# PriviligedLearningDistributedAerial/imitation

Hardware: AMD Instinct MI355X
Metric: env-steps/sec (whole node) + final eval return, GAIL HalfCheetah-v4 at 1/2/4/8 MI355X (higher is better)
Workload: dtype mixed (fp32 master weights and accumulation; PPO products as split-bf16 x3 ~fp32, discriminator bf16); 1 GPU; model=GAIL: FeedForward32Policy[32,32]+RunningNorm / BasicRewardNet(32,32)+RunningNorm, global_batch=4096, seq_len=512, parallelism=dp1, engine=device, env=HalfCheetah-v4

## Files before the change

csrc/bind/engine.cpp:

```cpp
#include "common.h"
#include "launchers.h"
#include "vec_env.h"

namespace {

template <typename T>
T* tptr(const py::dict& d, const char* k, bool optional = false) {
  if (!d.contains(k) || d[k].is_none()) {
    TORCH_CHECK(optional, "engine arg missing: ", k);
    return nullptr;
  }
  auto t = d[k].cast<torch::Tensor>();
  TORCH_CHECK(t.is_cuda() && t.is_contiguous(), "engine arg ", k, " must be a contiguous GPU tensor");
  return reinterpret_cast<T*>(t.data_ptr());
}

int ival(const py::dict& d, const char* k, int def = 0) { return d.contains(k) ? d[k].cast<int>() : def; }
double fval(const py::dict& d, const char* k, double def = 0.0) { return d.contains(k) ? d[k].cast<double>() : def; }

ia::WaveMLP wave_mlp(const py::dict& d) {
  ia::WaveMLP m{};
  auto Ws = d["W"].cast<std::vector<torch::Tensor>>();
  auto bs = d["b"].cast<std::vector<torch::Tensor>>();
  TORCH_CHECK(!Ws.empty() && Ws.size() <= (size_t)ia::kWaveMaxLayers, "1..4 layers");
// ... 280 lines not shown
  return o;
}

std::string ppo_row(py::dict d) {
  ia::PPORcPlan plan;
  return ppo_plan_rc(d, plan) ? std::string(plan.row->name) : "lds";
}

size_t ppo_lds(py::dict d) { return ia::ppo_lds_bytes(ppo_shape_args(d)); }

torch::Tensor ppo_image_probe(torch::Tensor x, int mode) {
  TORCH_CHECK(x.is_cuda() && x.scalar_type() == torch::kFloat32 && x.dim() == 2 && x.is_contiguous(),
              "engine_ppo_image_probe: a contiguous fp32 [rows][features] device matrix");
  const int rows = (int)x.size(0), feats = (int)x.size(1);
  TORCH_CHECK(rows > 0 && rows <= 64 && rows % 16 == 0 && feats > 0 && feats <= 64 && feats % 16 == 0,
              "engine_ppo_image_probe: rows and features multiples of 16, at most 64");
  TORCH_CHECK(mode == 0 || mode == 1, "engine_ppo_image_probe: mode 0 (packed store) or 1 (per element)");
  auto out = torch::zeros({2, feats / 16, (rows > 32 ? 64 : 32) / 32, 64, 8}, x.options().dtype(torch::kInt16));
  IA_HIP_CHECK(ia::ppo_image_probe_launch(x.data_ptr<float>(), rows, feats, mode,
                                           reinterpret_cast<unsigned short*>(out.data_ptr<int16_t>()), ia_stream()));
  return out;
}

}

void dagger_env_step(py::dict d) {
  ia::DaggerEnvArgs a{};
  std::string env = d["env"].cast<std::string>();
  int ms = 0;
  TORCH_CHECK(ia::make_env_params(env, &a.P, &ms), "unknown native env ", env);
  a.N = ival(d, "N");
  a.max_steps = ival(d, "max_steps", ms);
  a.mode = ival(d, "mode", 0);
  a.sdim = ia::state_size(a.P);
  a.state = tptr<float>(d, "state");
  a.rng = tptr<uint64_t>(d, "rng");
  a.elapsed = tptr<int>(d, "elapsed");
  a.ep_ret = tptr<float>(d, "ep_ret");
  auto check_numel = [&](const char* k, int64_t want) {
    if (!d.contains(k) || d[k].is_none()) return;
    auto t = d[k].cast<torch::Tensor>();
    TORCH_CHECK(t.numel() == want, "dagger_env_step: ", k, " has ", t.numel(), " elements, expected ", want);
  };
  check_numel("state", (int64_t)a.N * a.sdim);
  check_numel("rng", a.N);
  check_numel("elapsed", a.N);
// ... 25 lines not shown
    for (const char* k : {"rew", "term", "trunc", "ep_ret_out", "ep_len_out"}) check_numel(k, a.N);
    if (d.contains("obs_rec") && !d["obs_rec"].is_none()) {
      a.obs_rec = img ? (void*)tptr<uint8_t>(d, "obs_rec") : (void*)tptr<float>(d, "obs_rec");
      check_numel("obs_rec", a.N * obs_elems);
    }
  }
  IA_HIP_CHECK(ia::dagger_env_step(a, ia_stream()));
}

void register_engine(py::module& m) {
  m.def("dagger_env_step", &dagger_env_step, "DAgger collector: one device env step (mode 0) / reset all (mode 1)");
  m.def("engine_rollout", &rollout, "T-step device rollout (actor sampling + env) for N envs");
  m.def("engine_rollout_post", &rollout_post,
        "values, log-probs, TimeLimit bootstrap and learned reward of a rollout, all transitions in parallel");
  m.def("engine_reward_outnorm", &reward_outnorm, "NormalizedRewardNet output normalisation over a rollout");
  m.def("engine_reward_retnorm", &reward_retnorm, "VecNormalize discounted-return reward normalisation over a rollout");
  m.def("engine_ppo_update", &ppo_update, "persistent PPO update / DP minibatch grads / apply");
  m.def("engine_ppo_path", &ppo_path, "kernel used by engine_ppo_update mode 0 (rc | lds)");
  m.def("engine_ppo_row", &ppo_row, "instance-table row that engine_ppo_update mode 0 runs (lean or full; lds off the fast path)");
  m.def("engine_ppo_plan", &ppo_plan, "host plan of the register-chained PPO update: instance + launch geometry");
  m.def("engine_ppo_lds", &ppo_lds, "LDS bytes the PPO kernel needs for a configuration");
  m.def("engine_ppo_image_probe", &ppo_image_probe,
        "dW operand fragments of a matrix through the PPO update's split-bf16 image store and transposed reads (test hook)");
}
```

csrc/include/ia/wave.h:

```cpp
#pragma once
#include <hip/hip_runtime.h>
#include <stdint.h>

#include "ia/common.h"
#include "ia/mfma.h"
#include "ia/rng.h"

namespace ia {

typedef __attribute__((address_space(3))) float lf;
typedef float f32v4 __attribute__((ext_vector_type(4)));
typedef __attribute__((address_space(3))) f32v4 lf4;
typedef __attribute__((address_space(3))) int li;

__device__ __forceinline__ void wave_sync() {
  __builtin_amdgcn_fence(__ATOMIC_RELEASE, "wavefront");
  __builtin_amdgcn_wave_barrier();
  __builtin_amdgcn_fence(__ATOMIC_ACQUIRE, "wavefront");
}

__device__ __forceinline__ float bcast(float v, int k) {
  return __int_as_float(__builtin_amdgcn_readlane(__float_as_int(v), k));
}


template <int CTRL>
__device__ __forceinline__ float dpp(float v) {
  return __int_as_float(__builtin_amdgcn_update_dpp(0, __float_as_int(v), CTRL, 0xF, 0xF, true));
}
__device__ __forceinline__ float sum_lanes8(float v) {
  v += dpp<0xB1>(v);
  v += dpp<0x4E>(v);
  v += dpp<0x114>(v);
  return bcast(v, 7);
}

__device__ __forceinline__ float row_sum16(float v) {
  v += dpp<0xB1>(v);
  v += dpp<0x4E>(v);
  v += dpp<0x141>(v);
  v += dpp<0x140>(v);
  return v;
}
__device__ __forceinline__ float row_max16(float v) {
  v = fmaxf(v, dpp<0xB1>(v));
  v = fmaxf(v, dpp<0x4E>(v));
  v = fmaxf(v, dpp<0x141>(v));
  v = fmaxf(v, dpp<0x140>(v));
  return v;
}

__device__ __forceinline__ float add_rows16(float v) {
  const auto r = __builtin_amdgcn_permlane16_swap(__float_as_uint(v), __float_as_uint(v), false, false);
  return __uint_as_float(r[0]) + __uint_as_float(r[1]);
}
__device__ __forceinline__ float max_rows16(float v) {
  const auto r = __builtin_amdgcn_permlane16_swap(__float_as_uint(v), __float_as_uint(v), false, false);
  return fmaxf(__uint_as_float(r[0]), __uint_as_float(r[1]));
}
__device__ __forceinline__ float max_halves(float v) {
  const auto r = __builtin_amdgcn_permlane32_swap(__float_as_uint(v), __float_as_uint(v), false, false);
  return fmaxf(__uint_as_float(r[0]), __uint_as_float(r[1]));
}

__device__ __forceinline__ float add_halves(float v) {
  const auto r = __builtin_amdgcn_permlane32_swap(__float_as_uint(v), __float_as_uint(v), false, false);
// ... 28 lines not shown
```

csrc/kernels/launchers.h:

```cpp
#pragma once
#include <hip/hip_runtime.h>
#include <stddef.h>
#include <stdint.h>

#include "ia/engine.h"
#include "ia/tmlp.h"

namespace ia {

int tmlp_waves_for(const MLPDesc& d, int static_lds = 0);
size_t tmlp_slab_floats(const MLPDesc& d, int B);
hipError_t tmlp_forward(const MLPDesc& d, const float* X, int B, float* Y, hipStream_t s);
hipError_t tmlp_backward(const MLPDesc& d, const float* X, const float* dY, int B, float* dX, const MLPGrads& g,
                         float* slab, hipStream_t s);

int tmlp_disc_blocks(const MLPDesc& d, int B);
hipError_t tmlp_disc_fwd_bwd(const MLPDesc& d, const float* X, int B, const DiscLoss& dl, float* slab, hipStream_t s);

struct TransitionSrc {
  const float *obs, *next_obs, *acts;
  const int64_t* acts_i;
  const bool* dones;
};
struct RewardInputLayout {
// ... 382 lines not shown

bool rollout_split_form(const WaveMLP& m);
size_t rollout_lds_bytes(const RolloutArgs& a);
hipError_t rollout_launch(const RolloutArgs& a, hipStream_t s);
size_t rollout_post_lds_bytes(const RolloutPostArgs& a);
hipError_t rollout_post_launch(const RolloutPostArgs& a, hipStream_t s);
hipError_t reward_outnorm_launch(const OutNormArgs& a, hipStream_t s);
struct RetNormArgs {
  int T, N;
  const float* env_rew;
  const float* dones;
  const float* boot;
  float* rewards;
  double* ret;
  double* rms;
  double* work;
  double gamma, eps, clip;
};
hipError_t reward_retnorm_launch(const RetNormArgs& a, hipStream_t s);

bool ppo_rc_plan(const PPOArgs& a, PPORcPlan& plan);
hipError_t ppo_rc_launch(const PPOArgs& a, const PPORcPlan& plan, float* workspace, hipStream_t s);
hipError_t ppo_image_probe_launch(const float* x, int rows, int feats, int mode, unsigned short* out, hipStream_t s);

size_t ppo_lds_bytes(const PPOArgs& a);
hipError_t ppo_launch(const PPOArgs& a, hipStream_t s);

struct ConvGeo {
  int B, H, W, C;
  int KH, KW, S;
  int OH, OW, N;
  int P;
  int Kp;
};
bool conv_geo_ok(const ConvGeo& g);
constexpr int kMaxPack = 8;
struct ConvPackLayer {
  const float* w;
  void* wb;
  void* wt;
  int N, C, KH, KW;
  int t_hwc;
};
struct ConvPackArgs {
  ConvPackLayer layer[kMaxPack];
  int n;
// ... 80 lines not shown
```

csrc/kernels/ppo_rc.hip:

```cpp
#include <stdio.h>

#include "ppo_rc_kernel.h"
#include "ppo_rc_instances.h"

namespace ia {
namespace rc {

IA_RC_TABLE(IA_RC_EXTERN)

constexpr int kPrepWaves = 16;
constexpr int kPrepBatch = 16;

__device__ __forceinline__ int prep_idx(const PPOArgs& a, const PPORcGeo& g, int e, int mb, int c, int lane) {
  const int Bg = g.G * g.nch * g.cw;
  return a.perm[(size_t)e * a.rows + (size_t)mb * Bg + (size_t)c * g.cw + lane];
}

__global__ __launch_bounds__(64 * kPrepWaves) void ppo_rc_prep_kernel(PPOArgs a, PPORcGeo g) {
  __shared__ float red[kPrepWaves][64];
  __shared__ float stat[2][64];
  __shared__ float adv_stat[2];
  __shared__ float red_a[kPrepWaves];
  const int k = blockIdx.x;
  const int lane = threadIdx.x & 63, wv = threadIdx.x >> 6, nw = blockDim.x >> 6;
// ... 129 lines not shown
        bf16x4 hi, lo;
        split4(v, hi, lo);
        img_store4(L, 0, rp, t, st, hi, lo);
      }
    } else {
      for (int s = 0; s < feats / 4; ++s) img_store1(L, 0, rp, 4 * s + kk, row, x[(size_t)row * feats + 4 * s + kk]);
    }
  }
  __syncthreads();
  int t0, t1;
  img_lane_terms(r16, kk, t0, t1);
  const int n = T * ksteps;
  for (int i = gw; i < n; i += 4) {
    const int t = i / ksteps, ks = i - t * ksteps;
    const lch* p = (const lch*)L + t * img_strip(rp) + kImgKStep * ks + t0;
    const bf16x8 hi = img_read8(p, p + (t1 - t0));
    const bf16x8 lo = img_read8(p + img_lo(rp), p + img_lo(rp) + (t1 - t0));
    bf16x8* oh = reinterpret_cast<bf16x8*>(out) + (size_t)i * 64 + lane;
    oh[0] = hi;
    oh[(size_t)n * 64] = lo;
  }
}

}

using namespace rc;

hipError_t ppo_image_probe_launch(const float* x, int rows, int feats, int mode, unsigned short* out, hipStream_t s) {
  if (rows <= 0 || rows > kProbeMaxRows || rows % 16 != 0 || feats <= 0 || feats > kProbeMaxFeats || feats % 16 != 0 ||
      (mode != 0 && mode != 1))
    return hipErrorInvalidValue;
  hipLaunchKernelGGL(ppo_image_probe_kernel, dim3(1), dim3(256), 0, s, x, rows, feats, mode, out);
  return hipGetLastError();
}

static const PPORcRow kRcRows[] = {IA_RC_TABLE(IA_RC_ROW)};

static bool rc_row_bf3(const PPORcRow& r) { return rc_is_bf3(r.KT, r.S0T, r.NLT, r.HWT, r.CWT, r.NW); }

static const PPORcRow* rc_select(const PPOArgs& a, int kt, int cw, bool ns, bool bf3_ok, bool lean_ok) {
  const int s0 = (a.D + 3) / 4;
  for (const PPORcRow& r : kRcRows) {
    bool ok = r.ns == (int)ns && r.KT == kt && (r.CWT <= 0 || r.CWT == cw) && (lean_ok || !r.LEAN);
    ok = ok && (r.NLT <= 0 || (a.n_pi == r.NLT && a.n_vf == r.NLT));
    if (r.HWT > 0) {
      for (int l = 1; l < a.n_pi; ++l) ok = ok && a.pi_dims[l] == r.HWT;
      for (int l = 1; l < a.n_vf; ++l) ok = ok && a.vf_dims[l] == r.HWT;
    }
    ok = ok && (r.S0T > 0 ? s0 == r.S0T : (r.S0T == 0 || s0 <= -r.S0T));
// ... 228 lines not shown
```

csrc/kernels/ppo_rc_kernel.h:

```cpp
#pragma once
#include <hip/hip_runtime.h>
#include <stdlib.h>

#include "ia/engine.h"
#include "ia/wave.h"
#include "launchers.h"


namespace ia {
namespace rc {


typedef float f4 __attribute__((ext_vector_type(4)));
typedef __bf16 bf16;
typedef __bf16 bf16x8 __attribute__((ext_vector_type(8)));
typedef __attribute__((address_space(3))) bf16 lbf;
typedef __attribute__((address_space(3))) bf16x8 lbf8;
typedef __attribute__((address_space(3))) float lf;
typedef __attribute__((address_space(3))) f4 lf4;

constexpr int kL = kWaveMaxLayers;

__device__ __forceinline__ f4 mfma(float a, float b, f4 c) { return __builtin_amdgcn_mfma_f32_16x16x4f32(a, b, c, 0, 0, 0); }
__device__ __forceinline__ int rfl(int v) { return __builtin_amdgcn_readfirstlane(v); }
// ... 2 lines not shown
  const float e = __expf(2.f * fminf(fmaxf(x, -15.f), 15.f));
  return 1.f - 2.f * __builtin_amdgcn_rcpf(e + 1.f);
}

__device__ __forceinline__ float act_fn(int act, float x) {
  switch (act) {
    case 1: return fmaxf(x, 0.f);
    case 2: return tanh_fast(x);
    case 3: return x > 0.f ? x : 0.01f * x;
    case 4: return 1.f / (1.f + expf(-x));
    default: return x;
  }
}
__device__ __forceinline__ float act_grad(int act, float y) {
  switch (act) {
    case 1: return y > 0.f ? 1.f : 0.f;
    case 2: return 1.f - y * y;
    case 3: return y > 0.f ? 1.f : 0.01f;
    case 4: return y * (1.f - y);
    default: return 1.f;
  }
}
__device__ __forceinline__ float sum16(float v) { return row_sum16(v); }
__device__ __forceinline__ float sum_kk(float v) { return add_halves(add_rows16(v)); }
__device__ __forceinline__ float max_kk(float v) { return max_halves(max_rows16(v)); }

__device__ __forceinline__ void st_sc1_x4(float* p, f4 v) {
  asm volatile("global_store_dwordx4 %0, %1, off sc1" ::"v"(p), "v"(v) : "memory");
}
__device__ __forceinline__ void st_sc1_x1(float* p, float v) {
  asm volatile("global_store_dword %0, %1, off sc1" ::"v"(p), "v"(v) : "memory");
}
__device__ __forceinline__ f4 ld_sc1_x4(const float* p) {
  f4 v;
  asm volatile("global_load_dwordx4 %0, %1, off sc1" : "=v"(v) : "v"(p) : "memory");
  return v;
}
__device__ __forceinline__ void wait_vm4(f4& a, f4& b, f4& c, f4& d) {
  asm volatile("s_waitcnt vmcnt(0)" : "+v"(a), "+v"(b), "+v"(c), "+v"(d)::"memory");
}
__device__ __forceinline__ void wait_vm8(f4 (&v)[8]) {
  asm volatile("s_waitcnt vmcnt(0)"
               : "+v"(v[0]), "+v"(v[1]), "+v"(v[2]), "+v"(v[3]), "+v"(v[4]), "+v"(v[5]), "+v"(v[6]), "+v"(v[7])::"memory");
}
template <int N>
__device__ __forceinline__ void wait_vm_n(f4 (&v)[N]) {
// ... 25 lines not shown
__device__ __forceinline__ void spin_give_up(const PPOArgs& a, unsigned* tflag) {
  atomicOr(tflag, 1u);
  if (a.err) atomicOr(a.err, 1u);
}

struct LG {
  int din, dout, w, ldw, b, h, ldh, z, ldz, db;
};
__device__ __forceinline__ LG lg(const PPORcGeo& g, int q, int l) {
  LG r;
  r.din = rfl(g.din[q][l]);
  r.dout = rfl(g.dout[q][l]);
  r.w = rfl(g.w_off[q][l]);
  r.ldw = rfl(g.ldw[q][l]);
  r.b = rfl(g.b_off[q][l]);
  r.h = rfl(g.h_off[q][l]);
  r.ldh = rfl(g.ldh[q][l]);
  r.z = rfl(g.z_off[q][l]);
  r.ldz = rfl(g.ldz[q][l]);
  r.db = rfl(g.db_off[q][l]);
  return r;
}

template <int S0M>
struct Rows {
  float x[S0M];
  f4 act;
  f4 rd;
};

template <int S0M>
__device__ __forceinline__ void load_rows(const PPORcGeo& g, size_t slot, int row, int kk, int s0, Rows<S0M>& r) {
  const float* xr = g.xraw + (slot * 64 + row) * g.dp;
#pragma unroll
  for (int s = 0; s < S0M; ++s)
    if (s < s0) r.x[s] = xr[4 * s + kk];
  const float* ac = g.acts + (slot * 64 + row) * 16;
  r.act = *reinterpret_cast<const f4*>(ac + 4 * kk);
  r.rd = *reinterpret_cast<const f4*>(g.rowd + (slot * 64 + row) * 4);
}

template <int GT, int KI, int NF = 16>
__device__ __forceinline__ void exchange_sum(const float* slab, int n_items, const int (&ids)[KI], int lane, f4 (&xg)[KI]) {
  constexpr int IB0 = NF / GT;
  constexpr int IB = IB0 < KI ? IB0 : KI;
#pragma unroll
// ... 42 lines not shown
    if (rid[r] < 0) continue;
    f4 sacc = v[r * GT];
#pragma unroll
    for (int gi = 1; gi < GT; ++gi) sacc += v[r * GT + gi];
    st_sc1_x4(red + (size_t)rid[r] * 256 + lane * 4, sacc);
  }
}

typedef __bf16 bf16x4 __attribute__((ext_vector_type(4)));
typedef __attribute__((address_space(3))) bf16x4 lbf4;
typedef __attribute__((address_space(3))) char lch;

__host__ __device__ __forceinline__ int img_lo(int rp) { return 32 * rp; }
__host__ __device__ __forceinline__ int img_strip(int rp) { return 64 * rp; }
__host__ __device__ __forceinline__ int img_unit(int row, int p) {
  return 32 * (row ^ ((row >> 1) & 4)) + 8 * (p ^ ((row >> 2) & 3));
}
__device__ __forceinline__ void img_lane_terms(int r16, int kk, int& t0, int& t1) {
  t0 = img_unit(8 * kk + (r16 >> 2), r16 & 3);
  t1 = img_unit(8 * kk + 4 + (r16 >> 2), r16 & 3);
}
constexpr int kImgKStep = 32 * 32;

__device__ __forceinline__ void split4(const f4 v, bf16x4& hi, bf16x4& lo) {
#pragma clang fp contract(off)
#pragma unroll
  for (int j = 0; j < 4; ++j) {
    const bf16 h = (bf16)v[j];
    hi[j] = h;
    lo[j] = (bf16)(v[j] - (float)h);
  }
}
__device__ __forceinline__ bf16x8 cat4(bf16x4 a, bf16x4 b) { return __builtin_shufflevector(a, b, 0, 1, 2, 3, 4, 5, 6, 7); }

__device__ __forceinline__ void img_store4(lf* L, int off, int rp, int t, int st, bf16x4 hi, bf16x4 lo) {
  lch* p = (lch*)L + 4 * off + t * img_strip(rp) + st;
  *(lbf4*)p = hi;
  *(lbf4*)(p + img_lo(rp)) = lo;
}
__device__ __forceinline__ void img_store1(lf* L, int off, int rp, int f, int row, float v) {
  lch* p = (lch*)L + 4 * off + (f >> 4) * img_strip(rp) + img_unit(row, (f >> 2) & 3) + 2 * (f & 3);
  const bf16 h = (bf16)v;
  *(lbf*)p = h;
  *(lbf*)(p + img_lo(rp)) = (bf16)(v - (float)h);
}
__device__ __forceinline__ bf16x8 img_read8(const lch* a0, const lch* a1) {
  const bf16x4 x = __builtin_amdgcn_ds_read_tr16_b64_v4bf16((lbf4*)a0);
  const bf16x4 y = __builtin_amdgcn_ds_read_tr16_b64_v4bf16((lbf4*)a1);
  return cat4(x, y);
}

__device__ __forceinline__ f4 mfma_bf16(bf16x8 a, bf16x8 b, f4 c) { return __builtin_amdgcn_mfma_f32_16x16x32_bf16(a, b, c, 0, 0, 0); }

template <int N>
// ... 10 lines not shown
        const lch* zp = Lb + izo[i0 + i] + kImgKStep * ks;
        const lch* hp = Lb + iho[i0 + i] + kImgKStep * ks;
        zh[i] = img_read8(zp, zp + d1);
        zl[i] = img_read8(zp + lo, zp + lo + d1);
        hh[i] = img_read8(hp, hp + d1);
        hl[i] = img_read8(hp + lo, hp + lo + d1);
      }
#pragma unroll
      for (int i = 0; i < GS; ++i) {
        if (i0 + i >= N) continue;
        acc[i0 + i] = mfma_bf16(zh[i], hh[i], acc[i0 + i]);
        acc[i0 + i] = mfma_bf16(zh[i], hl[i], acc[i0 + i]);
        acc[i0 + i] = mfma_bf16(zl[i], hh[i], acc[i0 + i]);
      }
    }
  }
}

__host__ __device__ __forceinline__ int bf3_ld(int k) { return k + 8; }
__device__ __forceinline__ int bf3_pos_in0(int f) { return 8 * (f & 3) + (f >> 2); }
__device__ __forceinline__ int bf3_pos_h(int f) { return 32 * (f >> 5) + 8 * ((f >> 2) & 3) + 4 * ((f >> 4) & 1) + (f & 3); }

__device__ __forceinline__ void split8(const float (&v)[8], bf16x8& hi, bf16x8& lo) {
#pragma unroll
  for (int j = 0; j < 8; ++j) {
    const bf16 h = (bf16)v[j];
    hi[j] = h;
    lo[j] = (bf16)(v[j] - (float)h);
  }
}

__device__ __forceinline__ f4 bf3_tile(const lbf* a, int lo_off, bf16x8 bh, bf16x8 bl, f4 acc) {
  const bf16x8 ah = *(const lbf8*)a;
  const bf16x8 al = *(const lbf8*)(a + lo_off);
  acc = mfma_bf16(ah, bh, acc);
  acc = mfma_bf16(ah, bl, acc);
  return mfma_bf16(al, bh, acc);
}

__device__ __forceinline__ f4 bf3_mm(bf16x8 ah, bf16x8 al, bf16x8 bh, bf16x8 bl, f4 acc) {
  acc = mfma_bf16(ah, bh, acc);
  acc = mfma_bf16(ah, bl, acc);
  return mfma_bf16(al, bh, acc);
}

template <int KT>
__device__ __forceinline__ void bf3_store_w(lf* L, const PPORcGeo& g, int q, int l, int o, int i, float v, int nl) {
  const bf16 h = (bf16)v;
  const bf16 lo = (bf16)(v - (float)h);
  const int kin = l == 0 ? 32 : 16 * KT;
  const int rows = (g.dout[q][l] + 15) & ~15;
  lbf* wf = (lbf*)(L + g.wf_off[q][l]) + o * bf3_ld(kin) + (l == 0 ? bf3_pos_in0(i) : bf3_pos_h(i));
  wf[0] = h;
  wf[rows * bf3_ld(kin)] = lo;
  if (l > 0) {
    const int kout = l == nl - 1 ? 32 : 16 * KT;
    const int trows = (g.din[q][l] + 15) & ~15;
    lbf* wt = (lbf*)(L + g.wt_off[q][l]) + i * bf3_ld(kout) + bf3_pos_h(o);
    wt[0] = h;
    wt[trows * bf3_ld(kout)] = lo;
  }
}

template <int KT>
__device__ __forceinline__ void bf3_store_tile(lf* L, int kind, int wf, int wfl, int wt, int wtl, int r16, int kk,
                                               const float (&v)[4]) {
  typedef __bf16 bf16x4 __attribute__((ext_vector_type(4)));
  typedef __attribute__((address_space(3))) bf16x4 lbf4;
  bf16x4 h4, l4;
#pragma unroll
  for (int j = 0; j < 4; ++j) {
    const bf16 h = (bf16)v[j];
    h4[j] = h;
    l4[j] = (bf16)(v[j] - (float)h);
  }
  lbf* Lb = (lbf*)L;
  const int ldi = kind == 0 ? bf3_ld(32) : bf3_ld(16 * KT);
  lbf* pf = Lb + wf + 4 * kk * ldi + (kind == 0 ? 8 * (r16 & 3) + (r16 >> 2) : 8 * (r16 >> 2) + (r16 & 3));
#pragma unroll
  for (int j = 0; j < 4; ++j) {
    pf[j * ldi] = h4[j];
    pf[j * ldi + wfl] = l4[j];
  }
  if (kind != 0) {
    const int ldo = kind == 2 ? bf3_ld(32) : bf3_ld(16 * KT);
    lbf* pt = Lb + wt + r16 * ldo + 8 * kk;
    *(lbf4*)pt = h4;
    *(lbf4*)(pt + wtl) = l4;
  }
}

constexpr bool rc_is_bf3(int KT, int S0T, int NLT, int HWT, int CWT, int NW) {
  return HWT == 16 * KT && NLT == 3 && S0T != 0 && (S0T > 0 ? S0T : -S0T) <= 8 && CWT == 64 && (NW == 4 || KT == 2);
}

template <int KT, int KW, int KB, int S0T, int NLT, int ACTT, int HWT, int CWT, int DT, int NW, int LEAN = 0>
__global__ __launch_bounds__(64 * NW) void ppo_rc_kernel(PPOArgs a, PPORcGeo g) {
  constexpr int KI = KW + KB;
// ... 8 lines not shown
  const int w = rfl(tid >> 6), lane = tid & 63;
  const int r16 = lane & 15, kk = lane >> 4;
  const bool ns = g.ns != 0;
  int bid = (int)blockIdx.x;
  if (g.xcd > 1) {
    if (bid % g.xcd) return;
    bid /= g.xcd;
  }
  const int q = ns ? (bid & 1) : w / kHalf;
  const int gw = ns ? w : w % kHalf;
  const int grp = ns ? (bid >> 1) : bid;
  const int G = kLean ? 1 : g.G, nch = g.nch, cw = CWT > 0 ? CWT : g.cw;
  const int CH = G * nch;
  const int Bg = CH * cw;
  const int RT = cw / 16;
  const bool rows_wave = gw < RT;
  const int nl = NLT > 0 ? NLT : (q == 0 ? a.n_pi : a.n_vf);
  const int D = a.D, A = a.A;
  constexpr int S0M = S0T > 0 ? S0T : (S0T < 0 ? -S0T : 16);
  const int s0 = S0T > 0 ? S0T : (D + 3) / 4;
  constexpr bool BF3 = rc_is_bf3(KT, S0T, NLT, HWT, CWT, NW);
  constexpr bool kOffPath = KB == 1 && NW == 4;
  constexpr bool kNormBatch = kOffPath && S0T > 0 && KW <= 8;
  const bool gauss = DT >= 0 ? DT == 0 : !a.discrete;
  const bool has_ls = gauss && a.log_std_off >= 0;
  float am[4];
#pragma unroll
  for (int j = 0; j < 4; ++j) am[j] = 4 * (lane >> 4) + j < a.A ? 1.f : 0.f;
  const int n_mb = a.rows / Bg;
  const int K = a.n_epochs * n_mb;
  const float invB = 1.f / (float)Bg;
  const float c_half_log2pi = 0.91893853320467274f;
  const int n_items = rfl(g.n_items);

  for (int i = tid; i < g.lds_floats; i += kThreads) L[i] = 0.f;
  __syncthreads();
#pragma unroll
  for (int qq = 0; qq < 2; ++qq) {
#pragma unroll
    for (int l = 0; l < kL; ++l) {
      if (l >= (qq == 0 ? a.n_pi : a.n_vf) || (ns && qq != q)) continue;
      const LG y = lg(g, qq, l);
      const int wo = qq == 0 ? a.pi_w_off[l] : a.vf_w_off[l];
      const int bo = qq == 0 ? a.pi_b_off[l] : a.vf_b_off[l];
      for (int i = tid; i < y.dout * y.din; i += kThreads) {
        const int o = i / y.din, c = i - o * y.din;
// ... 157 lines not shown
    if (w + ib * kWaves >= nbq) continue;
    const int desc = rfl(g.items[bb + w + ib * kWaves]);
    const int iq = desc & 1, il = (desc >> 1) & 3, kind = (desc >> 3) & 3;
    const LG y = lg(g, iq, il);
    bkind[ib] = kind;
    b_off[ib] = kind == 1 ? y.db : g.lsp_off;
    const bool ok = kind == 1 ? (lane < y.dout) : (has_ls && lane < A);
    b_okf[ib] = ok ? 1.f : 0.f;
    if (ok) b_addr[ib] = kind == 1 ? y.b + lane : g.ls_off + lane;
  }
  float pre_m = 0.f, pre_v = 0.f;
  constexpr int kAhead = kOffPath ? 2 : 1;
  if (norm_lane && K > kAhead) {
    pre_m = g.mom[kAhead * 128 + nc];
    pre_v = g.mom[kAhead * 128 + 64 + nc];
  }
  Rows<S0M> cur;
  const int row = 16 * gw + r16;
  const int sterm = img_unit(row, kk);
  auto slot_of = [&](int u) -> size_t { return (size_t)(u / nch) * CH + (size_t)grp * nch + (u % nch); };
  if (rows_wave && K > 0) load_rows(g, slot_of(0), row, kk, s0, cur);
  __shared__ unsigned long long sprof[20];
  if (tid < 20) sprof[tid] = 0;
  unsigned* arrive = g.sync + (ns ? 4 * q : 0);
  unsigned* tflag = g.sync + 1;
  unsigned* arrive2 = g.sync + (ns ? 4 * q + 2 : 2);
  const unsigned spin_lim = a.spin_limit ? a.spin_limit : (1u << 22);
  const bool stall = a.debug_stall != 0 && bid == (ns ? 2 * G : G) - 1;
  __syncthreads();

  auto norm_rows = [&](int nbuf, float (&xo)[S0M]) {
    float nmv[S0M], nrv[S0M];
#pragma unroll
    for (int s = 0; s < S0M; ++s) {
      if constexpr (kNormBatch) {
        nmv[s] = L[g.nm_off + nbuf + 4 * s + kk];
        nrv[s] = L[g.nm_off + nbuf + 64 + 4 * s + kk];
      } else {
        nmv[s] = 0.f;
        nrv[s] = 1.f;
        if (s < s0 && a.has_norm) {
          nmv[s] = L[g.nm_off + nbuf + 4 * s + kk];
          nrv[s] = L[g.nm_off + nbuf + 64 + 4 * s + kk];
        }
      }
    }
#pragma unroll
    for (int s = 0; s < S0M; ++s) xo[s] = s < s0 ? (cur.x[s] - nmv[s]) * nrv[s] : 0.f;
    if (q == 0 || ns) {
      const int h0 = rfl(g.h_off[0][0]);
#pragma unroll
      for (int s = 0; s < S0M; ++s)
        if (s < s0) img_store1(L, h0, rp, 4 * s + kk, row, xo[s]);
    }
  };
  constexpr bool PREC = KW <= 8;
  const bool pre = PREC && (ns || G > 1) && (kLean || g.xstash < 0);
  float xpre[PREC ? S0M : 1];
#pragma unroll
  for (int s = 0; s < (PREC ? S0M : 1); ++s) xpre[s] = 0.f;
  auto pre_rows = [&](int k) {
    if constexpr (PREC)
      if (pre && rows_wave && k + 1 < K) norm_rows(((k + 1) & 1) * 128, xpre);
  };

  constexpr bool kEarly = KW <= 8;
  float step_size = 0.f, inv_bc2s = 0.f;
  auto adam_scalars = [&]() {
    step += 1.f;
    b1t *= a.beta1;
    b2t *= a.beta2;
    step_size = a.lr / (1.f - b1t);
    inv_bc2s = 1.f / sqrtf(1.f - b2t);
  };

  constexpr bool PREF = BF3 && KT == 2 && NW == 4;
  constexpr int PL = PREF ? NLT : 1, PT = PREF ? KT : 1;
  bf16x8 pwf[PL][PT][2], pwt[PL][PT][2];
  f4 pbs[PL][PT];
  f4 pls = {0.f, 0.f, 0.f, 0.f};

  const bool ent_wave = kOffPath && gauss && grp == 0 && (!ns || q == 0) && w == kWaves - 1;
  float ent_sl = 0.f;

  for (int k = 0; k < K; ++k) {
    unsigned long long t0 = prof ? clock64() : 0;
    const int nb = (k & 1) * 128;
    if constexpr (PREF) {
      if (rows_wave) {
// ... 244 lines not shown
            float sel = 0.f, ent = 0.f;
#pragma unroll
            for (int j = 0; j < 4; ++j) {
              const int o = 4 * kk + j;
              if (o < n) {
                lpk[j] = hv[j] - mx - lz;
                pk[j] = expf(lpk[j]);
                ent -= pk[j] * lpk[j];
                if (o == act_row) sel = lpk[j];
              }
            }
            logp = sum_kk(sel);
            ent_row = sum_kk(ent);
          }
          const float lr_ = logp - old_lp;
          const float ratio = expf(lr_);
          const float lo = 1.f - a.clip_range, hi = 1.f + a.clip_range;
          const float pl1 = adv * ratio, pl2 = adv * fminf(fmaxf(ratio, lo), hi);
          float c1, c2;
          if (pl1 < pl2) { c1 = 1.f; c2 = 0.f; } else if (pl2 < pl1) { c1 = 0.f; c2 = 1.f; } else { c1 = 0.5f; c2 = 0.5f; }
          const float inside = (ratio >= lo && ratio <= hi) ? 1.f : 0.f;
          const float dlogp = -invB * (c1 * adv + c2 * adv * inside) * ratio;
          if (gauss) {
            float lsp[4];
#pragma unroll
            for (int j = 0; j < 4; ++j) {
              const int o = 4 * kk + j;
              dzv[j] = dlogp * zs[j] * isd[j];
              lsp[j] = am[j] * dlogp * (zs[j] * zs[j] - 1.f);
            }
#pragma unroll
            for (int j = 0; j < 4; ++j) {
              const float s = sum16(lsp[j]);
              if (r16 == 0) L[g.lsp_off + gw * 16 + 4 * kk + j] = s;
            }
          } else {
#pragma unroll
            for (int j = 0; j < 4; ++j) {
              const int o = 4 * kk + j;
              dzv[j] = o < yh.dout ? dlogp * ((o == act_row ? 1.f : 0.f) - pk[j]) -
                                         a.ent_coef * invB * (-pk[j] * (lpk[j] + ent_row))
                                   : 0.f;
            }
          }
          dz = {dzv[0], dzv[1], dzv[2], dzv[3]};
          if (kk == 0) {
            st_pg += -fminf(pl1, pl2);
            st_cf += fabsf(ratio - 1.f) > a.clip_range ? 1.f : 0.f;
            st_kl += (ratio - 1.f) - lr_;
            if (!gauss) st_ent += -ent_row;
          }
        } else {
          float d = 0.f;
          if (kk == 0) {
            d = head.x - cur.rd.z;
            st_vl += d * d;
          }
          dz = {kk == 0 ? a.vf_coef * 2.f * d * invB : 0.f, 0.f, 0.f, 0.f};
        }
        unsigned long long c3 = prof ? clock64() : 0;
        f4 dzc[KT];
        dzc[0] = dz;
#pragma unroll
        for (int t = 1; t < KT; ++t) dzc[t] = {0.f, 0.f, 0.f, 0.f};
#pragma unroll
        for (int l = kL - 1; l >= 0; --l) {
          if (l >= nl) continue;
          const LG y = LY(l);
          const int tout = l == nl - 1 ? 1 : (HWT > 0 ? HWT / 16 : ((y.dout + 15) >> 4));
          const int tin = HWT > 0 ? HWT / 16 : ((y.din + 15) >> 4);
          constexpr int KWT = KT > 2 ? 1 : KT;
          float wt[KWT][KWT][4];
          if (!BF3 && KT <= 2 && l > 0) {
#pragma unroll
            for (int u2 = 0; u2 < KT; ++u2)
#pragma unroll
              for (int tt = 0; tt < KT; ++tt)
#pragma unroll
                for (int j = 0; j < 4; ++j)
                  if (u2 < tin && tt < tout) wt[u2 % KWT][tt % KWT][j] = L[y.w + (16 * tt + 4 * kk + j) * y.ldw + 16 * u2 + r16];
          }
          bf16x4 zsp[KT][2];
#pragma unroll
          for (int u2 = 0; u2 < KT; ++u2) zsp[u2][0] = zsp[u2][1] = bf16x4{(bf16)0.f, (bf16)0.f, (bf16)0.f, (bf16)0.f};
#pragma unroll
          for (int u2 = 0; u2 < KT; ++u2) {
            if (u2 >= tout) continue;
            split4(dzc[u2], zsp[u2][0], zsp[u2][1]);
            img_store4(L, y.z, rp, u2, sterm, zsp[u2][0], zsp[u2][1]);
            const float s0v = sum16(dzc[u2].x), s1v = sum16(dzc[u2].y), s2v = sum16(dzc[u2].z), s3v = sum16(dzc[u2].w);
            if (r16 == 0) {
              const f4 sv = {s0v, s1v, s2v, s3v};
              *(lf4*)(L + y.db + gw * 64 + 16 * u2 + 4 * kk) = sv;
            }
          }
          if (l == 0) break;
          f4 accb[KT];
#pragma unroll
          for (int u2 = 0; u2 < KT; ++u2) accb[u2] = {0.f, 0.f, 0.f, 0.f};
          if constexpr (BF3) {
            constexpr int KS = KT / 2;
            const bool head = l == nl - 1;
            const int ks_l = head ? 1 : KS;
            const int kout = head ? 32 : 16 * KT;
            const int trows = (y.din + 15) & ~15;
            const lbf* wt_img = (const lbf*)(L + WT(l)) + r16 * bf3_ld(kout) + 8 * kk;
#pragma unroll
            for (int ks = 0; ks < KS; ++ks) {
              if (ks >= ks_l) continue;
              const bf16x8 bh = cat4(zsp[2 * ks][0], zsp[2 * ks + 1][0]), bl = cat4(zsp[2 * ks][1], zsp[2 * ks + 1][1]);
#pragma unroll
              for (int u2 = 0; u2 < KT; ++u2) {
                if (u2 >= tin) continue;
                if constexpr (PREF) accb[u2] = bf3_mm(pwt[PREF ? l : 0][PREF ? u2 : 0][0], pwt[PREF ? l : 0][PREF ? u2 : 0][1], bh, bl, accb[u2]);
                else accb[u2] = bf3_tile(wt_img + 16 * u2 * bf3_ld(kout) + 32 * ks, trows * bf3_ld(kout), bh, bl, accb[u2]);
              }
            }
// ... 7 lines not shown
                  if (u2 < tin && tt < tout) accb[u2] = mfma(wt[u2 % KWT][tt % KWT][j], dzc[tt][j], accb[u2]);
          } else {
#pragma unroll
            for (int u2 = 0; u2 < KT; ++u2) {
              if (u2 >= tin) continue;
#pragma unroll
              for (int tt = 0; tt < KT; ++tt) {
                if (tt >= tout) continue;
                const lf* wc = L + y.w + (16 * tt + 4 * kk) * y.ldw + 16 * u2 + r16;
                accb[u2] = mfma(wc[0], dzc[tt].x, accb[u2]);
                accb[u2] = mfma(wc[y.ldw], dzc[tt].y, accb[u2]);
                accb[u2] = mfma(wc[2 * y.ldw], dzc[tt].z, accb[u2]);
                accb[u2] = mfma(wc[3 * y.ldw], dzc[tt].w, accb[u2]);
              }
            }
          }
          f4 nd[KT];
#pragma unroll
          for (int u2 = 0; u2 < KT; ++u2) {
            nd[u2] = {0.f, 0.f, 0.f, 0.f};
            if (u2 >= tin) continue;
            const f4 acc = accb[u2];
            const f4 hv = hreg[l > 0 ? l - 1 : 0][u2];
            nd[u2].x = acc.x * act_grad(hid_act, hv.x);
            nd[u2].y = acc.y * act_grad(hid_act, hv.y);
            nd[u2].z = acc.z * act_grad(hid_act, hv.z);
            nd[u2].w = acc.w * act_grad(hid_act, hv.w);
          }
#pragma unroll
          for (int u2 = 0; u2 < KT; ++u2) dzc[u2] = nd[u2];
        }
        if (prof && lane == 0 && gw == 0) {
          const unsigned long long c4 = clock64();
          const int pb = q == 1 ? 7 : 3;
          sprof[pb + 0] += c1 - c0;
          sprof[pb + 1] += c2 - c1;
          sprof[pb + 2] += c3 - c2;
          sprof[pb + 3] += c4 - c3;
        }
      }
      const unsigned long long cb0 = prof ? clock64() : 0;
      __syncthreads();
      const unsigned long long cb1 = prof ? clock64() : 0;
      if constexpr (!kOffPath)
        if (ch == 0 && norm_lane && k + 1 < K) norm_merge(mom_m, mom_v, 128 - nb);
      if (ent_wave) {
        f4 e4[4];
#pragma unroll
        for (int i = 0; i < 4; ++i) e4[i] = *(const lf4*)(L + g.ls_off + 4 * i);
        float sl = 0.f;
// ... 215 lines not shown
    for (int it = 0; it < KW; ++it) {
      if (it >= nwi) continue;
#pragma unroll
      for (int j = 0; j < 4; ++j) ss += gg[it][j] * gg[it][j];
    }
#pragma unroll
    for (int ib = 0; ib < KB; ++ib) {
      if (bkind[ib] < 0) continue;
      if (bkind[ib] == 2) bg[ib] -= a.ent_coef * b_okf[ib];
      ss += bg[ib] * bg[ib];
    }
    ss = wave_sum(ss);
    if (lane == 0) L[g.red_off + w] = ss;
    if constexpr (kOffPath) {
      if (ent_wave && lane == 0) {
        const float sl = ent_sl;
        st_ent += -(sl + A * (0.5f + c_half_log2pi));
      }
    } else if (gauss && tid == 0 && grp == 0 && q == 0) {
      float sl = 0.f;
      for (int j = 0; j < A; ++j) sl += has_ls ? L[g.ls_off + j] : 0.f;
      st_ent += -(sl + A * (0.5f + c_half_log2pi));
    }
    if (kEarly && !ns) adam_scalars();
    __syncthreads();
    unsigned long long t2 = prof ? clock64() : 0;

    float tot = 0.f;
#pragma unroll
    for (int i = 0; i < kWaves; ++i) tot += L[g.red_off + i];
    if (ns) {
      const unsigned long long x0 = prof ? clock64() : 0;
      unsigned long long* xs = reinterpret_cast<unsigned long long*>(g.sync + 8);
      const unsigned long long tag = (unsigned long long)(unsigned)(k + 1) << 32;
      if (tid == 0 && !stall) __hip_atomic_store(xs + q, tag | __float_as_uint(tot), __ATOMIC_RELAXED, __HIP_MEMORY_SCOPE_AGENT);
      unsigned long long o = 0;
      if (kEarly && tid == 0) o = __hip_atomic_load(xs + (1 - q), __ATOMIC_RELAXED, __HIP_MEMORY_SCOPE_AGENT);
      if (G == 1) pre_rows(k);
      if (kEarly) adam_scalars();
      if (tid == 0) {
        if (!kEarly) o = __hip_atomic_load(xs + (1 - q), __ATOMIC_RELAXED, __HIP_MEMORY_SCOPE_AGENT);
        unsigned spins = 0;
        while ((o >> 32) != (unsigned long long)(unsigned)(k + 1)) {
          __builtin_amdgcn_s_sleep(1);
          if (++spins > spin_lim || ld_sc1u(tflag) != 0u) {
            spin_give_up(a, tflag);
            break;
          }
          o = __hip_atomic_load(xs + (1 - q), __ATOMIC_RELAXED, __HIP_MEMORY_SCOPE_AGENT);
        }
        const float other = __uint_as_float((unsigned)(o & 0xffffffffu));
        L[g.red_off + 48] = q == 0 ? tot + other : other + tot;
      }
      __syncthreads();
      tot = L[g.red_off + 48];
      if (prof && tid == 0) sprof[16] += clock64() - x0;
    }
    constexpr bool kProfAdam = KW <= 8;
    if (kProfAdam && prof && tid == 0) sprof[17] -= clock64();
    if (!kEarly) adam_scalars();
    const float coef = fminf(1.f, a.max_grad_norm / (sqrtf(tot) + 1e-6f));
    const float b1 = a.beta1, b2 = a.beta2, eps = a.adam_eps;
// ... 57 lines not shown
      if (norm_lane) {
        norm_merge(pre_m, pre_v, nb);
        if (k + 3 < K) {
          pre_m = g.mom[(size_t)(k + 3) * 128 + nc];
          pre_v = g.mom[(size_t)(k + 3) * 128 + 64 + nc];
        }
      }
    }
    if (kProfAdam && prof && tid == 0) {
      const unsigned long long a1 = clock64();
      sprof[17] += a1;
      sprof[18] -= a1;
    }
    __syncthreads();
    if (prof && tid == 0) {
      const unsigned long long t3 = clock64();
      sprof[0] += t1 - t0;
      sprof[1] += t2 - t1;
      sprof[2] += t3 - t2;
      if (kProfAdam) sprof[18] += t3;
    }
  }

  const float vals[5] = {st_ent, st_pg, st_vl, st_cf, st_kl};
#pragma unroll
  for (int i = 0; i < 5; ++i) {
    const float v = wave_sum(vals[i]);
    if (lane == 0) L[g.red_off + 8 + w * 5 + i] = v;
  }
  __syncthreads();
  if (tid < 5) {
    float s = 0.f;
    for (int i = 0; i < kWaves; ++i) s += L[g.red_off + 8 + i * 5 + tid];
    if (!(tid == 0 && gauss)) s *= invB;
    if (G > 1 || ns) atomicAdd(a.stats + tid, s);
    else a.stats[tid] += s;
  }
  if (grp != 0) return;
  const bool shared_wb = !ns || q == 0;

#pragma unroll
  for (int qq = 0; qq < 2; ++qq) {
#pragma unroll
    for (int l = 0; l < kL; ++l) {
      if (l >= (qq == 0 ? a.n_pi : a.n_vf) || (ns && qq != q)) continue;
      const LG y = lg(g, qq, l);
// ... 58 lines not shown
```

Baseline: 1.875 million env-steps/s.

## Fuse PPO row sums, vectorize bf16 splits, precompute Adam bias-correction table

Several micro-optimizations land in the register-chained PPO update kernel. Four independent 16-lane row sums are batched into one inline-asm DPP sequence, and on the off path the first reduction step is folded into an fma of the factors. The split-bf16 hi/lo conversions now use packed two-wide conversions, and the per-step Adam bias-correction scalars come from a shared-memory table filled once at kernel start instead of being recomputed each minibatch step. The changes target ALU and latency overhead inside the inner update loop. They add LDS use, hand-written asm that needs correct s_nop hazard handling, and a small numerical change from the fused fma and the table's accumulated powers. A probe binding for testing is also added.

```diff
diff --git a/csrc/bind/engine.cpp b/csrc/bind/engine.cpp
--- a/csrc/bind/engine.cpp
+++ b/csrc/bind/engine.cpp
@@ -326,6 +326,17 @@
   return out;
 }
 
+torch::Tensor ppo_rowsum_probe(torch::Tensor a, torch::Tensor b, int mode) {
+  for (const torch::Tensor& t : {a, b})
+    TORCH_CHECK(t.is_cuda() && t.scalar_type() == torch::kFloat32 && t.dim() == 2 && t.size(0) == 64 && t.size(1) == 4 &&
+                    t.is_contiguous(),
+                "engine_ppo_rowsum_probe: contiguous fp32 [64][4] device matrices");
+  TORCH_CHECK(mode == 0 || mode == 1, "engine_ppo_rowsum_probe: mode 0 (plain sums) or 1 (first step an fma of the factors)");
+  auto out = torch::zeros_like(a);
+  IA_HIP_CHECK(ia::ppo_rowsum_probe_launch(a.data_ptr<float>(), b.data_ptr<float>(), mode, out.data_ptr<float>(), ia_stream()));
+  return out;
+}
+
 }
 
 void dagger_env_step(py::dict d) {
@@ -397,4 +408,5 @@
   m.def("engine_ppo_lds", &ppo_lds, "LDS bytes the PPO kernel needs for a configuration");
   m.def("engine_ppo_image_probe", &ppo_image_probe,
         "dW operand fragments of a matrix through the PPO update's split-bf16 image store and transposed reads (test hook)");
-}
+  m.def("engine_ppo_rowsum_probe", &ppo_rowsum_probe, "one wave's fused four-value row sums of the PPO update (test hook)");
+}
diff --git a/csrc/include/ia/wave.h b/csrc/include/ia/wave.h
--- a/csrc/include/ia/wave.h
+++ b/csrc/include/ia/wave.h
@@ -42,6 +42,26 @@
   v += dpp<0x140>(v);
   return v;
 }
+#define IA_ROW_ADD4(ctrl)                                                   \
+  "v_add_f32_dpp %0, %0, %0 " ctrl " row_mask:0xf bank_mask:0xf bound_ctrl:1\n\t" \
+  "v_add_f32_dpp %1, %1, %1 " ctrl " row_mask:0xf bank_mask:0xf bound_ctrl:1\n\t" \
+  "v_add_f32_dpp %2, %2, %2 " ctrl " row_mask:0xf bank_mask:0xf bound_ctrl:1\n\t" \
+  "v_add_f32_dpp %3, %3, %3 " ctrl " row_mask:0xf bank_mask:0xf bound_ctrl:1\n\t"
+__device__ __forceinline__ f32v4 row_sum16x4_tail(f32v4 v) {
+  float x = v.x, y = v.y, z = v.z, w = v.w;
+  asm("s_nop 1\n\t" IA_ROW_ADD4("quad_perm:[2,3,0,1]") IA_ROW_ADD4("row_half_mirror") IA_ROW_ADD4("row_mirror")
+      : "+v"(x), "+v"(y), "+v"(z), "+v"(w));
+  return f32v4{x, y, z, w};
+}
+__device__ __forceinline__ f32v4 row_sum16x4(f32v4 v) {
+  float x = v.x, y = v.y, z = v.z, w = v.w;
+  asm("s_nop 1\n\t" IA_ROW_ADD4("quad_perm:[1,0,3,2]") IA_ROW_ADD4("quad_perm:[2,3,0,1]") IA_ROW_ADD4("row_half_mirror")
+          IA_ROW_ADD4("row_mirror")
+      : "+v"(x), "+v"(y), "+v"(z), "+v"(w));
+  return f32v4{x, y, z, w};
+}
+#undef IA_ROW_ADD4
+
 __device__ __forceinline__ float row_max16(float v) {
   v = fmaxf(v, dpp<0xB1>(v));
   v = fmaxf(v, dpp<0x4E>(v));
diff --git a/csrc/kernels/launchers.h b/csrc/kernels/launchers.h
--- a/csrc/kernels/launchers.h
+++ b/csrc/kernels/launchers.h
@@ -428,6 +428,7 @@
 bool ppo_rc_plan(const PPOArgs& a, PPORcPlan& plan);
 hipError_t ppo_rc_launch(const PPOArgs& a, const PPORcPlan& plan, float* workspace, hipStream_t s);
 hipError_t ppo_image_probe_launch(const float* x, int rows, int feats, int mode, unsigned short* out, hipStream_t s);
+hipError_t ppo_rowsum_probe_launch(const float* a, const float* b, int mode, float* out, hipStream_t s);
 
 size_t ppo_lds_bytes(const PPOArgs& a);
 hipError_t ppo_launch(const PPOArgs& a, hipStream_t s);
diff --git a/csrc/kernels/ppo_rc.hip b/csrc/kernels/ppo_rc.hip
--- a/csrc/kernels/ppo_rc.hip
+++ b/csrc/kernels/ppo_rc.hip
@@ -175,9 +175,29 @@
   }
 }
 
+__global__ __launch_bounds__(64) void ppo_rowsum_probe_kernel(const float* a, const float* b, int mode, float* out) {
+  const int lane = threadIdx.x;
+  const f4 va = *reinterpret_cast<const f4*>(a + 4 * lane);
+  f4 r;
+  if (mode == 0) {
+    r = sum16x4(va);
+  } else {
+    const f4 vb = *reinterpret_cast<const f4*>(b + 4 * lane);
+    const f4 p = {va.x * vb.x, va.y * vb.y, va.z * vb.z, va.w * vb.w};
+    r = sum16x4_fma(va, vb, p);
+  }
+  *reinterpret_cast<f4*>(out + 4 * lane) = r;
+}
+
 }
 
 using namespace rc;
+
+hipError_t ppo_rowsum_probe_launch(const float* a, const float* b, int mode, float* out, hipStream_t s) {
+  if (mode != 0 && mode != 1) return hipErrorInvalidValue;
+  hipLaunchKernelGGL(ppo_rowsum_probe_kernel, dim3(1), dim3(64), 0, s, a, b, mode, out);
+  return hipGetLastError();
+}
 
 hipError_t ppo_image_probe_launch(const float* x, int rows, int feats, int mode, unsigned short* out, hipStream_t s) {
   if (rows <= 0 || rows > kProbeMaxRows || rows % 16 != 0 || feats <= 0 || feats > kProbeMaxFeats || feats % 16 != 0 ||
diff --git a/csrc/kernels/ppo_rc_kernel.h b/csrc/kernels/ppo_rc_kernel.h
--- a/csrc/kernels/ppo_rc_kernel.h
+++ b/csrc/kernels/ppo_rc_kernel.h
@@ -48,6 +48,15 @@
   }
 }
 __device__ __forceinline__ float sum16(float v) { return row_sum16(v); }
+__device__ __forceinline__ f4 sum16x4(f4 v) { return row_sum16x4(v); }
+__device__ __forceinline__ f4 sum16x4_fma(f4 a, f4 b, f4 p) {
+  f4 s;
+  s.x = __builtin_fmaf(a.x, b.x, dpp<0xB1>(p.x));
+  s.y = __builtin_fmaf(a.y, b.y, dpp<0xB1>(p.y));
+  s.z = __builtin_fmaf(a.z, b.z, dpp<0xB1>(p.z));
+  s.w = __builtin_fmaf(a.w, b.w, dpp<0xB1>(p.w));
+  return row_sum16x4_tail(s);
+}
 __device__ __forceinline__ float sum_kk(float v) { return add_halves(add_rows16(v)); }
 __device__ __forceinline__ float max_kk(float v) { return max_halves(max_rows16(v)); }
 
@@ -119,6 +128,20 @@
   return r;
 }
 
+constexpr int kAdamTab = 512;
+__device__ __forceinline__ void adam_tab_fill(float2* tab, int K, int tid, int nthreads, float b1t, float b2t, float beta1,
+                                              float beta2, float lr) {
+#pragma clang fp contract(off)
+  for (int e = tid; e < K; e += nthreads) {
+    float p1 = b1t, p2 = b2t;
+    for (int i = 0; i <= e; ++i) {
+      p1 *= beta1;
+      p2 *= beta2;
+    }
+    tab[e] = make_float2(lr / (1.f - p1), 1.f / sqrtf(1.f - p2));
+  }
+}
+
 template <int S0M>
 struct Rows {
   float x[S0M];
@@ -207,14 +230,34 @@
 }
 constexpr int kImgKStep = 32 * 32;
 
+typedef __bf16 bf16x2 __attribute__((ext_vector_type(2)));
+typedef float f2 __attribute__((ext_vector_type(2)));
+__device__ __forceinline__ bf16x2 cvt_bf2(float a, float b) { return __builtin_convertvector(f2{a, b}, bf16x2); }
+__device__ __forceinline__ void bf2_floats(bf16x2 h, float& a, float& b) {
+  const unsigned u = __builtin_bit_cast(unsigned, h);
+  a = __uint_as_float(u << 16);
+  b = __uint_as_float(u & 0xffff0000u);
+}
+__device__ __forceinline__ void split2(float a, float b, bf16x2& hi, bf16x2& lo) {
+#pragma clang fp contract(off)
+  hi = cvt_bf2(a, b);
+  float ha, hb;
+  bf2_floats(hi, ha, hb);
+  lo = cvt_bf2(a - ha, b - hb);
+}
+__device__ __forceinline__ void split2c(float a, float b, bf16x2& hi, bf16x2& lo) {
+  hi = cvt_bf2(a, b);
+  float ha, hb;
+  bf2_floats(hi, ha, hb);
+  lo = cvt_bf2(a - ha, b - hb);
+}
+__device__ __forceinline__ bf16x4 cat2(bf16x2 a, bf16x2 b) { return __builtin_shufflevector(a, b, 0, 1, 2, 3); }
 __device__ __forceinline__ void split4(const f4 v, bf16x4& hi, bf16x4& lo) {
-#pragma clang fp contract(off)
-#pragma unroll
-  for (int j = 0; j < 4; ++j) {
-    const bf16 h = (bf16)v[j];
-    hi[j] = h;
-    lo[j] = (bf16)(v[j] - (float)h);
-  }
+  bf16x2 h0, l0, h1, l1;
+  split2(v.x, v.y, h0, l0);
+  split2(v.z, v.w, h1, l1);
+  hi = cat2(h0, h1);
+  lo = cat2(l0, l1);
 }
 __device__ __forceinline__ bf16x8 cat4(bf16x4 a, bf16x4 b) { return __builtin_shufflevector(a, b, 0, 1, 2, 3, 4, 5, 6, 7); }
 
@@ -271,12 +314,11 @@
 __device__ __forceinline__ int bf3_pos_h(int f) { return 32 * (f >> 5) + 8 * ((f >> 2) & 3) + 4 * ((f >> 4) & 1) + (f & 3); }
 
 __device__ __forceinline__ void split8(const float (&v)[8], bf16x8& hi, bf16x8& lo) {
-#pragma unroll
-  for (int j = 0; j < 8; ++j) {
-    const bf16 h = (bf16)v[j];
-    hi[j] = h;
-    lo[j] = (bf16)(v[j] - (float)h);
-  }
+  bf16x2 h[4], l[4];
+#pragma unroll
+  for (int j = 0; j < 4; ++j) split2c(v[2 * j], v[2 * j + 1], h[j], l[j]);
+  hi = cat4(cat2(h[0], h[1]), cat2(h[2], h[3]));
+  lo = cat4(cat2(l[0], l[1]), cat2(l[2], l[3]));
 }
 
 __device__ __forceinline__ f4 bf3_tile(const lbf* a, int lo_off, bf16x8 bh, bf16x8 bl, f4 acc) {
@@ -316,13 +358,10 @@
                                                const float (&v)[4]) {
   typedef __bf16 bf16x4 __attribute__((ext_vector_type(4)));
   typedef __attribute__((address_space(3))) bf16x4 lbf4;
-  bf16x4 h4, l4;
-#pragma unroll
-  for (int j = 0; j < 4; ++j) {
-    const bf16 h = (bf16)v[j];
-    h4[j] = h;
-    l4[j] = (bf16)(v[j] - (float)h);
-  }
+  bf16x2 h0, l0, h1, l1;
+  split2c(v[0], v[1], h0, l0);
+  split2c(v[2], v[3], h1, l1);
+  const bf16x4 h4 = cat2(h0, h1), l4 = cat2(l0, l1);
   lbf* Lb = (lbf*)L;
   const int ldi = kind == 0 ? bf3_ld(32) : bf3_ld(16 * KT);
   lbf* pf = Lb + wf + 4 * kk * ldi + (kind == 0 ? 8 * (r16 & 3) + (r16 >> 2) : 8 * (r16 >> 2) + (r16 & 3));
@@ -377,6 +416,7 @@
   constexpr bool BF3 = rc_is_bf3(KT, S0T, NLT, HWT, CWT, NW);
   constexpr bool kOffPath = KB == 1 && NW == 4;
   constexpr bool kNormBatch = kOffPath && S0T > 0 && KW <= 8;
+  constexpr bool kEarly = KW <= 8;
   const bool gauss = DT >= 0 ? DT == 0 : !a.discrete;
   const bool has_ls = gauss && a.log_std_off >= 0;
   float am[4];
@@ -580,6 +620,10 @@
   if (rows_wave && K > 0) load_rows(g, slot_of(0), row, kk, s0, cur);
   __shared__ unsigned long long sprof[20];
   if (tid < 20) sprof[tid] = 0;
+  __shared__ float2 adam_tab[kEarly ? kAdamTab : 1];
+  const bool use_tab = kEarly && K <= kAdamTab;
+  if constexpr (kEarly)
+    if (use_tab) adam_tab_fill(adam_tab, K, tid, kThreads, b1t, b2t, a.beta1, a.beta2, a.lr);
   unsigned* arrive = g.sync + (ns ? 4 * q : 0);
   unsigned* tflag = g.sync + 1;
   unsigned* arrive2 = g.sync + (ns ? 4 * q + 2 : 2);
@@ -622,7 +666,6 @@
       if (pre && rows_wave && k + 1 < K) norm_rows(((k + 1) & 1) * 128, xpre);
   };
 
-  constexpr bool kEarly = KW <= 8;
   float step_size = 0.f, inv_bc2s = 0.f;
   auto adam_scalars = [&]() {
     step += 1.f;
@@ -913,17 +956,28 @@
           const float inside = (ratio >= lo && ratio <= hi) ? 1.f : 0.f;
           const float dlogp = -invB * (c1 * adv + c2 * adv * inside) * ratio;
           if (gauss) {
-            float lsp[4];
+            float lsp[4], lsa[4], lsb[4];
 #pragma unroll
             for (int j = 0; j < 4; ++j) {
               const int o = 4 * kk + j;
               dzv[j] = dlogp * zs[j] * isd[j];
-              lsp[j] = am[j] * dlogp * (zs[j] * zs[j] - 1.f);
-            }
-#pragma unroll
-            for (int j = 0; j < 4; ++j) {
-              const float s = sum16(lsp[j]);
-              if (r16 == 0) L[g.lsp_off + gw * 16 + 4 * kk + j] = s;
+              lsa[j] = am[j] * dlogp;
+              lsb[j] = zs[j] * zs[j] - 1.f;
+              lsp[j] = lsa[j] * lsb[j];
+            }
+            if constexpr (kOffPath) {
+              const f4 s4 = sum16x4_fma(f4{lsa[0], lsa[1], lsa[2], lsa[3]}, f4{lsb[0], lsb[1], lsb[2], lsb[3]},
+                                        f4{lsp[0], lsp[1], lsp[2], lsp[3]});
+              if (r16 == 0) {
+#pragma unroll
+                for (int j = 0; j < 4; ++j) L[g.lsp_off + gw * 16 + 4 * kk + j] = s4[j];
+              }
+            } else {
+#pragma unroll
+              for (int j = 0; j < 4; ++j) {
+                const float s = sum16(lsp[j]);
+                if (r16 == 0) L[g.lsp_off + gw * 16 + 4 * kk + j] = s;
+              }
             }
           } else {
 #pragma unroll
@@ -951,6 +1005,7 @@
         }
         unsigned long long c3 = prof ? clock64() : 0;
         f4 dzc[KT];
+        f4 dza[kOffPath ? KT : 1], dzg[kOffPath ? KT : 1];
         dzc[0] = dz;
 #pragma unroll
         for (int t = 1; t < KT; ++t) dzc[t] = {0.f, 0.f, 0.f, 0.f};
@@ -979,11 +1034,14 @@
             if (u2 >= tout) continue;
             split4(dzc[u2], zsp[u2][0], zsp[u2][1]);
             img_store4(L, y.z, rp, u2, sterm, zsp[u2][0], zsp[u2][1]);
-            const float s0v = sum16(dzc[u2].x), s1v = sum16(dzc[u2].y), s2v = sum16(dzc[u2].z), s3v = sum16(dzc[u2].w);
-            if (r16 == 0) {
-              const f4 sv = {s0v, s1v, s2v, s3v};
-              *(lf4*)(L + y.db + gw * 64 + 16 * u2 + 4 * kk) = sv;
-            }
+            f4 sv;
+            if constexpr (kOffPath) {
+              if (l == nl - 1) sv = sum16x4(dzc[u2]);
+              else sv = sum16x4_fma(dza[kOffPath ? u2 : 0], dzg[kOffPath ? u2 : 0], dzc[u2]);
+            } else {
+              sv = f4{sum16(dzc[u2].x), sum16(dzc[u2].y), sum16(dzc[u2].z), sum16(dzc[u2].w)};
+            }
+            if (r16 == 0) *(lf4*)(L + y.db + gw * 64 + 16 * u2 + 4 * kk) = sv;
           }
           if (l == 0) break;
           f4 accb[KT];
@@ -1037,10 +1095,15 @@
             if (u2 >= tin) continue;
             const f4 acc = accb[u2];
             const f4 hv = hreg[l > 0 ? l - 1 : 0][u2];
-            nd[u2].x = acc.x * act_grad(hid_act, hv.x);
-            nd[u2].y = acc.y * act_grad(hid_act, hv.y);
-            nd[u2].z = acc.z * act_grad(hid_act, hv.z);
-            nd[u2].w = acc.w * act_grad(hid_act, hv.w);
+            const f4 ag = {act_grad(hid_act, hv.x), act_grad(hid_act, hv.y), act_grad(hid_act, hv.z), act_grad(hid_act, hv.w)};
+            nd[u2].x = acc.x * ag.x;
+            nd[u2].y = acc.y * ag.y;
+            nd[u2].z = acc.z * ag.z;
+            nd[u2].w = acc.w * ag.w;
+            if constexpr (kOffPath) {
+              dza[kOffPath ? u2 : 0] = acc;
+              dzg[kOffPath ? u2 : 0] = ag;
+            }
           }
 #pragma unroll
           for (int u2 = 0; u2 < KT; ++u2) dzc[u2] = nd[u2];
@@ -1302,13 +1365,20 @@
       for (int j = 0; j < A; ++j) sl += has_ls ? L[g.ls_off + j] : 0.f;
       st_ent += -(sl + A * (0.5f + c_half_log2pi));
     }
-    if (kEarly && !ns) adam_scalars();
+    if (kEarly && !ns && !use_tab) adam_scalars();
     __syncthreads();
     unsigned long long t2 = prof ? clock64() : 0;
 
     float tot = 0.f;
 #pragma unroll
     for (int i = 0; i < kWaves; ++i) tot += L[g.red_off + i];
+    if constexpr (kEarly) {
+      if (use_tab) {
+        const float2 ab = adam_tab[k];
+        step_size = ab.x;
+        inv_bc2s = ab.y;
+      }
+    }
     if (ns) {
       const unsigned long long x0 = prof ? clock64() : 0;
       unsigned long long* xs = reinterpret_cast<unsigned long long*>(g.sync + 8);
@@ -1317,7 +1387,7 @@
       unsigned long long o = 0;
       if (kEarly && tid == 0) o = __hip_atomic_load(xs + (1 - q), __ATOMIC_RELAXED, __HIP_MEMORY_SCOPE_AGENT);
       if (G == 1) pre_rows(k);
-      if (kEarly) adam_scalars();
+      if (kEarly && !use_tab) adam_scalars();
       if (tid == 0) {
         if (!kEarly) o = __hip_atomic_load(xs + (1 - q), __ATOMIC_RELAXED, __HIP_MEMORY_SCOPE_AGENT);
         unsigned spins = 0;
@@ -1421,6 +1491,7 @@
     }
   }
 
+  if (use_tab) step += (float)K;
   const float vals[5] = {st_ent, st_pg, st_vl, st_cf, st_kl};
 #pragma unroll
   for (int i = 0; i < 5; ++i) {
```

Result: faster. 1.959 million env-steps/s (median of 5 runs) (+4.5%).
